# kit-cel/vae-equalizer

Measured on NVIDIA B200. Metric: DP VAE-LE train symbols/s, higher is better.
Workload: dtype f32

## Files before the change

### include/vaeq.h

```cpp
#ifndef VAEQ_H_
#define VAEQ_H_

#include <stddef.h>
#include <stdint.h>

#ifdef __cplusplus
extern "C" {
#endif

#define VAEQ_ABI_VERSION 1

#define VAEQ_OK 0
#define VAEQ_EINVAL (-1)
#define VAEQ_EWORKSPACE (-2)
#define VAEQ_ENODEV (-3)

#define VAEQ_MAX_TAPS 63
#define VAEQ_MAX_LEVELS 8

int vaeq_abi_version(void);
const char *vaeq_last_error(void);
int vaeq_sm_count(void);

#define VAEQ_K_DP_FWD 0
// ... 7 lines not shown
#define VAEQ_K_DP_BWD2 8
#define VAEQ_K_DP_BWD3 9
#define VAEQ_K_DP_FRAME 10
#define VAEQ_NKINDS 11
int vaeq_kernel_timing(int32_t enable);
int vaeq_kernel_timing_read(float *ms_sum, int32_t *count);
int64_t vaeq_launch_count(int32_t kind);

typedef struct vaeq_dp_desc {
    int32_t B;
    int32_t sps;
    int32_t M;
    int32_t n_lev;
    float nu_sc;
    int32_t flags;
    const float *rx;
    int64_t ld_rx;
    const float *amp;
    const float *P;
    const float *var;
    float *W;
    float *h;
    float *adam;
    float *q;
    int64_t ld_q;
    float *out;
    int64_t ld_out;
    float *q_keep;
    int64_t ld_q_keep;
    float *out_keep;
    int64_t ld_out_keep;
    int32_t keep_lo, keep_n;
    float *loss;
    float *var_est;
    float *gW;
    float *gh;
    void *workspace;
    size_t workspace_bytes;
} vaeq_dp_desc;

#define VAEQ_F_AMSGRAD 1

size_t vaeq_dp_workspace_bytes(int32_t B, int32_t M, int32_t n_lev);
size_t vaeq_adam_state_floats(int32_t M);

int vaeq_dp_force_generic(int32_t on);

int vaeq_dp_dynamic_tiles(int32_t on);

int vaeq_dp_tc_taps(int32_t on);

int vaeq_dp_tc_forward(int32_t on);

int vaeq_dp_forward(const vaeq_dp_desc *d, void *stream);
int vaeq_dp_forward_backward(const vaeq_dp_desc *d, void *stream);
int vaeq_dp_loss_from_q(const vaeq_dp_desc *d, float *gq, int64_t ld_gq, void *stream);

size_t vaeq_eq_backward_scratch_bytes(int32_t B, int32_t M);
int vaeq_eq_backward(const float *rx, int64_t ld_rx, const float *q, int64_t ld_q, const float *out, int64_t ld_out, const float *gq,
                     int64_t ld_gq, const float *gout, int64_t ld_gout, const float *amp, const float *var, int32_t n_lev, int32_t B,
                     int32_t M, float *gW, void *scratch, void *stream);

int vaeq_dp_train_step(const vaeq_dp_desc *d, float lr_w, float lr_h, void *stream);

int vaeq_dp_train_frame(const vaeq_dp_desc *d, int32_t n_steps, int32_t stride_sym, int32_t keep_lo_in_dst,
                        float lr_w, float lr_h, float *loss_steps, float *var_est_steps, void *stream);

int vaeq_dp_persistent_frames(int32_t mode);

size_t vaeq_dp_runs_workspace_bytes(int32_t B, int32_t M, int32_t n_lev, int32_t n_runs);
typedef struct vaeq_dp_runs {
    int32_t n_runs;
    int64_t rs_rx, rs_amp, rs_P, rs_var, rs_W, rs_h, rs_adam, rs_q, rs_out, rs_q_keep, rs_out_keep;
    const float *nu_sc;
    const float *lr_w, *lr_h;
} vaeq_dp_runs;
int vaeq_dp_train_frame_runs(const vaeq_dp_desc *d, const vaeq_dp_runs *runs, int32_t n_steps, int32_t stride_sym,
                             int32_t keep_lo_in_dst, float lr_w, float lr_h, float *loss_steps, float *var_est_steps,
                             void *stream);
int vaeq_dp_frame_runs_per_sm(int32_t per_sm);

size_t vaeq_dp_split_stats_doubles(int32_t M);
int vaeq_dp_split_forward(const vaeq_dp_desc *d, int32_t sym_lo, int32_t sym_hi, double *stats_out, void *stream);
int vaeq_dp_split_backward(const vaeq_dp_desc *d, int32_t sym_lo, int32_t sym_hi, const double *stats_in, float *grads_out,
                           void *stream);
int vaeq_dp_split_update(const vaeq_dp_desc *d, const float *grads_in, float lr_w, float lr_h, void *stream);
#define VAEQ_MAX_PEERS 8
typedef struct vaeq_peer_comm {
    int32_t rank, world;
    void *slot[VAEQ_MAX_PEERS];
    int32_t *epoch;
} vaeq_peer_comm;
size_t vaeq_peer_slot_bytes(int32_t M);
int vaeq_dp_split_step_peer(const vaeq_dp_desc *d, int32_t sym_lo, int32_t sym_hi, const vaeq_peer_comm *comm, float lr_w, float lr_h,
                            void *stream);

int vaeq_adam_update(float *param, const float *grad, float *state, int32_t n, float lr, int32_t amsgrad,
                     int32_t *step_count, int32_t bump_step, void *stream);

int vaeq_soft_dec(const float *out, int64_t ld_out, const float *var, const float *amp, float nu_sc,
                  int32_t n_lev, int32_t N, float *q, int64_t ld_q, void *stream);

int vaeq_soft_dec_runs(const float *out, const float *var, const float *amp, const float *nu_sc, int32_t n_lev, int32_t N,
                       int32_t n_runs, float *q, void *stream);

size_t vaeq_find_shift_scratch_bytes(int32_t n_shift);
// ... 106 lines not shown
```

### vae_equalizer_b200/_lib.py

```python
from __future__ import annotations

import ctypes as C
import functools
import os

_HERE = os.path.dirname(os.path.abspath(__file__))
LIB_PATH = os.path.join(_HERE, "libvaeq.so")

c_f32p = C.POINTER(C.c_float)


class VaeqError(RuntimeError):
    pass


class DpDesc(C.Structure):
    _fields_ = [
        ("B", C.c_int32), ("sps", C.c_int32), ("M", C.c_int32), ("n_lev", C.c_int32),
        ("nu_sc", C.c_float), ("flags", C.c_int32),
        ("rx", C.c_void_p), ("ld_rx", C.c_int64),
        ("amp", C.c_void_p), ("P", C.c_void_p), ("var", C.c_void_p),
        ("W", C.c_void_p), ("h", C.c_void_p), ("adam", C.c_void_p),
        ("q", C.c_void_p), ("ld_q", C.c_int64),
        ("out", C.c_void_p), ("ld_out", C.c_int64),
# ... 5 lines not shown
        ("workspace", C.c_void_p), ("workspace_bytes", C.c_size_t),
    ]


class DpRuns(C.Structure):
    _fields_ = [
        ("n_runs", C.c_int32),
        ("rs_rx", C.c_int64), ("rs_amp", C.c_int64), ("rs_P", C.c_int64), ("rs_var", C.c_int64),
        ("rs_W", C.c_int64), ("rs_h", C.c_int64), ("rs_adam", C.c_int64), ("rs_q", C.c_int64), ("rs_out", C.c_int64),
        ("rs_q_keep", C.c_int64), ("rs_out_keep", C.c_int64),
        ("nu_sc", C.c_void_p), ("lr_w", C.c_void_p), ("lr_h", C.c_void_p),
    ]


class PeerComm(C.Structure):
    _fields_ = [("rank", C.c_int32), ("world", C.c_int32), ("slot", C.c_void_p * 8), ("epoch", C.c_void_p)]


class AwgnRuns(C.Structure):
    _fields_ = [
        ("n_runs", C.c_int32),
        ("rs_rx", C.c_int64), ("rs_W", C.c_int64), ("rs_h", C.c_int64), ("rs_adam", C.c_int64), ("rs_P", C.c_int64),
        ("rs_q", C.c_int64), ("rs_out", C.c_int64), ("rs_loss", C.c_int64),
        ("lr", C.c_void_p), ("var", C.c_void_p), ("amp_mean", C.c_void_p),
    ]


class AwgnDesc(C.Structure):
    _fields_ = [
        ("B", C.c_int32), ("sps", C.c_int32), ("M", C.c_int32), ("n_lev", C.c_int32),
        ("amp_mean", C.c_float), ("var", C.c_float),
        ("rx", C.c_void_p), ("amp", C.c_void_p), ("P", C.c_void_p),
        ("W", C.c_void_p), ("h", C.c_void_p), ("adam", C.c_void_p),
        ("q", C.c_void_p), ("out", C.c_void_p), ("loss", C.c_void_p),
        ("gW", C.c_void_p), ("gh", C.c_void_p),
        ("workspace", C.c_void_p), ("workspace_bytes", C.c_size_t),
    ]


_i32, _i64, _f, _vp, _sz, _u64 = C.c_int32, C.c_int64, C.c_float, C.c_void_p, C.c_size_t, C.c_uint64
PROTOTYPES = {
    "vaeq_abi_version": (C.c_int, []),
    "vaeq_last_error": (C.c_char_p, []),
    "vaeq_sm_count": (C.c_int, []),
    "vaeq_kernel_timing": (C.c_int, [_i32]),
    "vaeq_kernel_timing_read": (C.c_int, [_vp, _vp]),
    "vaeq_launch_count": (C.c_int64, [_i32]),
    "vaeq_dp_workspace_bytes": (_sz, [_i32, _i32, _i32]),
    "vaeq_adam_state_floats": (_sz, [_i32]),
    "vaeq_dp_force_generic": (C.c_int, [_i32]),
    "vaeq_dp_dynamic_tiles": (C.c_int, [_i32]),
    "vaeq_dp_tc_taps": (C.c_int, [_i32]),
    "vaeq_dp_tc_forward": (C.c_int, [_i32]),
    "vaeq_dp_forward": (C.c_int, [C.POINTER(DpDesc), _vp]),
    "vaeq_dp_forward_backward": (C.c_int, [C.POINTER(DpDesc), _vp]),
    "vaeq_dp_loss_from_q": (C.c_int, [C.POINTER(DpDesc), _vp, _i64, _vp]),
    "vaeq_eq_backward_scratch_bytes": (_sz, [_i32, _i32]),
    "vaeq_eq_backward": (C.c_int, [_vp, _i64, _vp, _i64, _vp, _i64, _vp, _i64, _vp, _i64, _vp, _vp, _i32, _i32, _i32, _vp, _vp, _vp]),
    "vaeq_dp_train_step": (C.c_int, [C.POINTER(DpDesc), _f, _f, _vp]),
    "vaeq_dp_train_frame": (C.c_int, [C.POINTER(DpDesc), _i32, _i32, _i32, _f, _f, _vp, _vp, _vp]),
    "vaeq_dp_persistent_frames": (C.c_int, [_i32]),
    "vaeq_dp_frame_runs_per_sm": (C.c_int, [_i32]),
    "vaeq_dp_runs_workspace_bytes": (_sz, [_i32, _i32, _i32, _i32]),
    "vaeq_dp_train_frame_runs": (C.c_int, [C.POINTER(DpDesc), C.POINTER(DpRuns), _i32, _i32, _i32, _f, _f, _vp, _vp, _vp]),
    "vaeq_dp_split_stats_doubles": (_sz, [_i32]),
    "vaeq_dp_split_forward": (C.c_int, [C.POINTER(DpDesc), _i32, _i32, _vp, _vp]),
    "vaeq_dp_split_backward": (C.c_int, [C.POINTER(DpDesc), _i32, _i32, _vp, _vp, _vp]),
    "vaeq_dp_split_update": (C.c_int, [C.POINTER(DpDesc), _vp, _f, _f, _vp]),
    "vaeq_peer_slot_bytes": (_sz, [_i32]),
    "vaeq_dp_split_step_peer": (C.c_int, [C.POINTER(DpDesc), _i32, _i32, C.POINTER(PeerComm), _f, _f, _vp]),
    "vaeq_adam_update": (C.c_int, [_vp, _vp, _vp, _i32, _f, _i32, _vp, _i32, _vp]),
    "vaeq_soft_dec": (C.c_int, [_vp, _i64, _vp, _vp, _f, _i32, _i32, _vp, _i64, _vp]),
    "vaeq_find_shift_scratch_bytes": (_sz, [_i32]),
    "vaeq_find_shift": (C.c_int, [_vp, _i64, _vp, _i64, _vp, _i64, _vp, _i32, _i32, _i32, _vp, _vp, _vp, _vp, _vp]),
    "vaeq_ser_iqflip": (C.c_int, [_vp, _i64, _vp, _i64, _i32, _i32, _vp, _vp, _vp]),
    "vaeq_ser_constell": (C.c_int, [_vp, _i64, _vp, _i64, _vp, _vp, _f, _i32, _i32, _vp, _vp, _vp, _vp]),
    "vaeq_frame_eval_scratch_bytes": (_sz, [_i32, _i32]),
    "vaeq_frame_eval_runs": (C.c_int, [_vp, _i64, _i64, _vp, _i64, _i64, _vp, _i64, _i64, _vp, _vp, _i64, _vp, _i32, _i32, _i32, _i32, _i32,
                                      _i32, _i32, _vp, _vp, _vp, _vp, _vp]),
    "vaeq_frame_eval_runs_ex": (C.c_int, [_vp, _i64, _i64, _vp, _i64, _i64, _vp, _i64, _i64, _vp, _vp, _i64, _vp, _i32, _i32, _i32, _i32, _i32,
                                         _i32, _i32, _i32, _vp, _vp, _vp, _vp, _vp, _vp]),
    "vaeq_cma_align_rescale": (C.c_int, [_vp, _i64, _i64, _vp, _vp, _i32, _i32, _i32, _vp, _vp]),
    "vaeq_soft_dec_runs": (C.c_int, [_vp, _vp, _vp, _vp, _i32, _i32, _i32, _vp, _vp]),
    "vaeq_gmi": (C.c_int, [_vp, _i64, _vp, _i64, _vp, _i32, _i32, _vp, _vp, _vp]),
    "vaeq_cma_scratch_bytes": (_sz, [_i32, _i32, _i32]),
    "vaeq_cma": (C.c_int, [_i32, _vp, _i32, _f, _vp, _i32, _f, _i32, _i32, _i32, _i32, _vp, _vp, _i32, _vp, _vp]),
    "vaeq_cpe_scratch_bytes": (_sz, [_i32]),
    "vaeq_gen_levels": (C.c_int, [_vp, _vp, _i32, _i32, _i32, _i32, _u64, _vp, _vp, _i32, _vp]),
    "vaeq_gen_pulse": (C.c_int, [_vp, _vp, _i32, _i32, _vp, _i32, _vp]),
    "vaeq_gen_jones": (C.c_int, [_vp, _vp, _vp, _vp, _f, _f, _i32, _i32, _vp]),
    "vaeq_gen_noise": (C.c_int, [_vp, _vp, _u64, _i32, _i32, _vp, _i32, _vp]),
    "vaeq_cpe": (C.c_int, [_vp, _i32, _vp, _vp, _vp]),
    "vaeq_cpe_runs_scratch_bytes": (_sz, [_i32, _i32]),
    "vaeq_cpe_runs": (C.c_int, [_vp, _i32, _i32, _vp, _vp, _vp]),
    "vaeq_cma_awgn": (C.c_int, [_vp, _i32, _f, _vp, _i32, _f, _i32, _i32, _vp, _vp, _i32, _vp]),
    "vaeq_cpe_awgn": (C.c_int, [_vp, _i32, _i32, _vp, _vp, _vp]),
    "vaeq_ser_cma": (C.c_int, [_vp, _i64, _vp, _i64, _vp, _i32, _i32, _vp, _vp, _vp, _vp]),
    "vaeq_find_shift_symb": (C.c_int, [_vp, _i32, _vp, _i64, _i32, _i32, _vp, _vp, _vp]),
    "vaeq_cma_awgn_runs": (C.c_int, [_vp, _i64, _i64, _i64, _i32, _i32, _vp, _i64, _i64, _i32, _vp, _i32, _vp, _f, _i32, _vp, _i32, _vp]),
    "vaeq_awgn_cma_eval_scratch_bytes": (_sz, [_i32, _i32, _i32, _i32]),
    "vaeq_awgn_cma_eval_runs": (C.c_int, [_vp, _i64, _i64, _vp, _i64, _i64, _vp, _i32, _i32, _i32, _i32, _i32, _vp, _vp, _vp, _vp, _vp]),
    "vaeq_awgn_workspace_bytes": (_sz, [_i32, _i32, _i32]),
    "vaeq_adam_state_floats_awgn": (_sz, [_i32]),
    "vaeq_awgn_forward": (C.c_int, [C.POINTER(AwgnDesc), _vp]),
    "vaeq_awgn_forward_backward": (C.c_int, [C.POINTER(AwgnDesc), _vp]),
    "vaeq_awgn_train_step": (C.c_int, [C.POINTER(AwgnDesc), _f, _f, _vp]),
# ... 71 lines not shown
```

### vae_equalizer_b200/csrc/dp_fast.cu

```cuda
#include "dp_fast.cuh"

namespace vaeq {

template <bool SWZ = false>
__device__ __forceinline__ void load_x_phases(const DpK &p, int t0, float4 *xe, float4 *xo) {
    const int sym0 = t0 - FT_HP - FT_XOFF;
#pragma unroll 1
    for (int j = threadIdx.x; j < FT_XN / 2; j += FT_NT) {
        const int64_t s0 = 2 * (int64_t)sym0 + 4 * j;
        float4 v[4];
        if (s0 >= 0 && s0 + 3 < p.L) {
#pragma unroll
            for (int r = 0; r < 4; ++r) v[r] = __ldg(reinterpret_cast<const float4 *>(p.rx + (int64_t)r * p.ld_rx + s0));
        } else {
#pragma unroll
            for (int r = 0; r < 4; ++r) {
                float t[4];
#pragma unroll
                for (int k = 0; k < 4; ++k) {
                    const int64_t s = s0 + k;
                    t[k] = (s >= 0 && s < p.L) ? p.rx[(int64_t)r * p.ld_rx + s] : 0.f;
                }
                v[r] = make_float4(t[0], t[1], t[2], t[3]);
            }
// ... 474 lines not shown
    }

#pragma unroll
    for (int a = 0; a < RL::AMAX; ++a)
#pragma unroll
        for (int k = 0; k < 8; ++k) {
            const float2 v2 = acc2[a][2 * (k >> 2) + (k & 1)];
            const float s = warp_sum(((k >> 1) & 1) ? v2.y : v2.x);
            if (lane == 0) red[wid * (RL::AMAX * 8) + a * 8 + k] = s;
        }
    __syncthreads();
    if (wid < 4) {
        float *dst = p.gpart + (int64_t)blockIdx.x * 16 * M;
        for (int idx = lane; idx < n_real * 8; idx += 32) {
            const int a = idx >> 3, k = idx & 7, oi = k >> 1, cidx = k & 1, o = oi >> 1, i = oi & 1;
            float s = 0.f;
            if (a == BASE) {
#pragma unroll
                for (int w = 0; w < FT_NW; ++w) s += red[w * (RL::AMAX * 8) + idx];
            } else {
#pragma unroll
                for (int w = wid; w < FT_NW; w += 4) s += red[w * (RL::AMAX * 8) + idx];
            }
            const int lag = a0 + a;
            if (FAM == 1) dst[8 * M + ((o * 2 + i) * 2 + cidx) * M + (2 * MH - ph - 2 * lag)] = 2.f * p.scal[DP_KAPPA_OFF + o] * s;
            else dst[(o * 4 + 2 * cidx + i) * M + (2 * lag + ph)] = s;
        }
    }
}

template <int MH>
static size_t fast_smem_fwd() {
    return (size_t)(2 * FT_XS + FT_ES + 2 * FT_TAPV * (2 * MH + 1) + FT_RAW) * sizeof(float4) + sizeof(FastConst) + 5 * 32 * sizeof(float) + 64;
}
template <int MH>
static size_t fast_smem_bwd1() {
    return (size_t)(2 * FT_ES + FT_TAPV * (2 * MH + 1) + 12 * FT_NT) * sizeof(float4) + sizeof(FastConst) + (2 * (2 * MH + 2) + 2) * sizeof(float) + 64;
}
template <int MH, int FAM>
static size_t fast_smem_taps() {
    return (size_t)(FAM == 0 ? 2 * FT_XS + FT_RAW + 2 * 4 * FT_GROW : FT_ES + 4 * FT_GROW + 2 * 8 * FT_GROW) * sizeof(float4) +
           FT_NW * Roles<MH>::AMAX * 8 * sizeof(float) + 64;
}

template <typename K>
static int fast_prepare(K kern, size_t smem, int *grid) {
    VAEQ_CUDA(cudaFuncSetAttribute(kern, cudaFuncAttributeMaxDynamicSharedMemorySize, (int)smem));
    int per = 0;
    VAEQ_CUDA(cudaOccupancyMaxActiveBlocksPerMultiprocessor(&per, kern, FT_NT, smem));
    *grid = max(1, per) * sm_count();
    return VAEQ_OK;
}

extern bool g_tc_taps, g_tc_fwd;
template <int NL, int MH>
static int dp_run_fast_t(DpK p, int mode, cudaStream_t st, int *grid_bwd_out) {
    static int grids[VAEQ_MAX_DEVICES][4] = {{0}};
    int &gF = grids[cur_device()][0], &g1 = grids[cur_device()][1], &g2 = grids[cur_device()][2], &g3 = grids[cur_device()][3];
    const size_t sf = fast_smem_fwd<MH>(), s1 = fast_smem_bwd1<MH>(), s2 = fast_smem_taps<MH, 0>(), s3 = fast_smem_taps<MH, 1>();
    if (!gF) {
        int rc;
        if ((rc = fast_prepare(k_dp_fwd_fast<NL, MH>, sf, &gF))) return rc;
        if ((rc = fast_prepare(k_dp_bwd1_fast<NL, MH>, s1, &g1))) return rc;
        if ((rc = fast_prepare(k_dp_taps_fast<MH, 0>, s2, &g2))) return rc;
        if ((rc = fast_prepare(k_dp_taps_fast<MH, 1>, s3, &g3))) return rc;
        g2 = g3 = min(g2, g3);
    }
    p.T = FT_T;
    p.keep_vec = p.qk != nullptr && p.keep_lo % 4 == 0 && p.keep_base % 4 == 0 && p.ld_qk % 4 == 0 && p.ld_outk % 4 == 0 &&
                 (reinterpret_cast<uintptr_t>(p.qk) | reinterpret_cast<uintptr_t>(p.outk)) % 16 == 0;
    const int nt_f = (p.chi - p.clo + FT_T - 1) / FT_T, nt_b = (p.sym_hi - p.sym_lo + FT_T - 1) / FT_T;
    const int gf = min(min(gF, DP_GRID_CAP), nt_f), gb1 = min(min(g1, DP_GRID_CAP), nt_b), gt = min(min(g2, DP_GRID_CAP), nt_b);
    if (mode != DP_MODE_SPLIT_BWD) {
        p.ntiles = nt_f;
        int nparts_f = gf, rc_f = VAEQ_OK;
        if (g_tc_fwd && dp_fwd_tc_launch(p, NL, st, &nparts_f, &rc_f)) {
            if (rc_f) return rc_f;
        } else {
            ktime_begin(VAEQ_K_DP_FWD, st);
            k_dp_fwd_fast<NL, MH><<<gf, FT_NT, sf, st>>>(p);
            ktime_end(VAEQ_K_DP_FWD, st);
            VAEQ_LAUNCH_CHECK("k_dp_fwd_fast");
        }
        *grid_bwd_out = nparts_f;
        if (mode == DP_MODE_SPLIT_FWD) return VAEQ_OK;
        const int rc = dp_launch_fin(p, nparts_f, st);
        if (rc) return rc;
    }
    if (mode == DP_MODE_FWD) return VAEQ_OK;
    p.ntiles = nt_b;
    ktime_begin(VAEQ_K_DP_BWD, st);
    k_dp_bwd1_fast<NL, MH><<<gb1, FT_NT, s1, st>>>(p);
    ktime_end(VAEQ_K_DP_BWD, st);
    VAEQ_LAUNCH_CHECK("k_dp_bwd1_fast");
    if (g_tc_taps) {
        int rc = VAEQ_OK;
        if (dp_taps_tc_launch(p, st, grid_bwd_out, &rc)) return rc;
    }
    ktime_begin(VAEQ_K_DP_BWD2, st);
    k_dp_taps_fast<MH, 0><<<gt, FT_NT, s2, st>>>(p);
    ktime_end(VAEQ_K_DP_BWD2, st);
    VAEQ_LAUNCH_CHECK("k_dp_taps_fast<W>");
    ktime_begin(VAEQ_K_DP_BWD3, st);
    k_dp_taps_fast<MH, 1><<<gt, FT_NT, s3, st>>>(p);
    ktime_end(VAEQ_K_DP_BWD3, st);
    VAEQ_LAUNCH_CHECK("k_dp_taps_fast<h>");
    *grid_bwd_out = gt;
    return VAEQ_OK;
}

bool g_tc_fwd = true;

bool g_tc_taps = true;

int dp_try_fast(const DpK &p, int n_lev, int mode, cudaStream_t st, int *grid_bwd_out, int *rc) {
    const bool no_q = p.q == nullptr;
    const bool aligned = (p.B % 4 == 0) && (p.ld_rx % 4 == 0) && (no_q || ((p.ld_q % 4 == 0) && (p.ld_out % 4 == 0))) &&
                         ((reinterpret_cast<uintptr_t>(p.rx) | reinterpret_cast<uintptr_t>(p.q) | reinterpret_cast<uintptr_t>(p.out)) % 16 == 0);
    if (!aligned || p.B < 2 * FT_T) return 0;
    if ((p.sym_lo | p.sym_hi | p.clo | p.chi) % 4 != 0) return 0;
    *rc = VAEQ_OK;
#define FAST_CASE(NL_, MH_)                                             \
    if (n_lev == NL_ && p.mh == MH_) {                                  \
        *rc = dp_run_fast_t<NL_, MH_>(p, mode, st, grid_bwd_out);       \
        return 1;                                                       \
    }
    FAST_CASE(8, 12)
    FAST_CASE(8, 6)
    FAST_CASE(8, 4)
    FAST_CASE(8, 2)
    FAST_CASE(4, 12)
    FAST_CASE(2, 12)
#undef FAST_CASE
    return 0;
}

}

extern "C" int vaeq_dp_tc_forward(int32_t on) {
    vaeq::g_tc_fwd = on != 0;
    return VAEQ_OK;
}

extern "C" int vaeq_dp_tc_taps(int32_t on) {
    if (on != 0 && on != 1) {
        vaeq::set_error("vaeq_dp_tc_taps: %d is not 0 (CUDA-core kernels) or 1 (tensor cores)", on);
        return VAEQ_EINVAL;
    }
    vaeq::g_tc_taps = on != 0;
    return VAEQ_OK;
}
```

### vae_equalizer_b200/csrc/dp_fwd_tc.cu

```cuda
#include <type_traits>
#include "dp_fast.cuh"
#include "tma.cuh"

namespace vaeq {

constexpr int FC_NG = 4;
constexpr int FC_GT = 128;
constexpr int FC_NT = FC_NG * FC_GT;
constexpr int FC_XCH = 264;
constexpr int FC_XCB = 4352;
constexpr int FC_XB = 4 * FC_XCB;
constexpr int FC_QB = 8704;
static_assert(2 * FC_QB <= FC_XB && FC_QB % 512 == 0 && FC_QB >= 528 * 16, "E_q hi | lo live in the x_lo array");
static_assert(FT_TE == 4 * FC_GT, "a tile is 128 blocks of 4 symbols");

__device__ __forceinline__ uint64_t umma_desc(uint32_t saddr, uint32_t lbo, uint32_t sbo, uint32_t layout) {
    return (uint64_t)((saddr >> 4) & 0x3fff) | ((uint64_t)((lbo >> 4) & 0x3fff) << 16) | ((uint64_t)((sbo >> 4) & 0x3fff) << 32) | (1ull << 46) |
           ((uint64_t)layout << 61);
}
constexpr uint32_t UMMA_SW_NONE = 0, UMMA_SW64 = 4, UMMA_SW32 = 6;
__host__ __device__ constexpr uint32_t umma_idesc_k(int N) { return (1u << 4) | (2u << 7) | (2u << 10) | ((uint32_t)(N >> 3) << 17) | ((128u >> 4) << 24); }
__device__ __forceinline__ void umma_tf32_k(uint32_t tmem_d, uint64_t da, uint64_t db, uint32_t idesc, uint32_t acc) {
    asm volatile(
        "{\n\t.reg .pred p;\n\tsetp.ne.b32 p, %4, 0;\n\t"
        "tcgen05.mma.cta_group::1.kind::tf32 [%0], %1, %2, %3, p;\n\t}\n" ::"r"(tmem_d),
        "l"(da), "l"(db), "r"(idesc), "r"(acc)
        : "memory");
}
__device__ __forceinline__ void umma_commit_to(uint64_t *bar) {
    asm volatile("tcgen05.commit.cta_group::1.mbarrier::arrive::one.shared::cluster.b64 [%0];" ::"r"(smem_u32(bar)) : "memory");
}
__device__ __forceinline__ float tf32_lo_part(float x) {
    const float r = x - __uint_as_float(__float_as_uint(x) & 0xffffe000u);
    uint32_t o;
    asm("cvt.rna.tf32.f32 %0, %1;" : "=r"(o) : "f"(r));
    return __uint_as_float(o);
}
__device__ __forceinline__ void tmem_ld16_issue(uint32_t taddr, float (&v)[16]) {
    asm volatile("tcgen05.ld.sync.aligned.32x32b.x16.b32 {%0,%1,%2,%3,%4,%5,%6,%7,%8,%9,%10,%11,%12,%13,%14,%15}, [%16];"
                 : "=f"(v[0]), "=f"(v[1]), "=f"(v[2]), "=f"(v[3]), "=f"(v[4]), "=f"(v[5]), "=f"(v[6]), "=f"(v[7]), "=f"(v[8]), "=f"(v[9]), "=f"(v[10]),
                   "=f"(v[11]), "=f"(v[12]), "=f"(v[13]), "=f"(v[14]), "=f"(v[15])
                 : "r"(taddr));
}
__device__ __forceinline__ void tmem_ld16_wait(float (&v)[16]) {
    asm volatile("tcgen05.wait::ld.sync.aligned;"
                 : "+f"(v[0]), "+f"(v[1]), "+f"(v[2]), "+f"(v[3]), "+f"(v[4]), "+f"(v[5]), "+f"(v[6]), "+f"(v[7]), "+f"(v[8]), "+f"(v[9]), "+f"(v[10]),
                   "+f"(v[11]), "+f"(v[12]), "+f"(v[13]), "+f"(v[14]), "+f"(v[15])
                 :
                 : "memory");
}
__device__ __forceinline__ void tmem_ld16(uint32_t taddr, float (&v)[16]) {
    tmem_ld16_issue(taddr, v);
    tmem_ld16_wait(v);
}
__device__ __forceinline__ void tmem_st16(uint32_t taddr, const float (&v)[16]) {
    asm volatile("tcgen05.st.sync.aligned.32x32b.x16.b32 [%0], {%1,%2,%3,%4,%5,%6,%7,%8,%9,%10,%11,%12,%13,%14,%15,%16};" ::"r"(taddr),
                 "r"(__float_as_uint(v[0])), "r"(__float_as_uint(v[1])), "r"(__float_as_uint(v[2])), "r"(__float_as_uint(v[3])), "r"(__float_as_uint(v[4])),
                 "r"(__float_as_uint(v[5])), "r"(__float_as_uint(v[6])), "r"(__float_as_uint(v[7])), "r"(__float_as_uint(v[8])), "r"(__float_as_uint(v[9])),
                 "r"(__float_as_uint(v[10])), "r"(__float_as_uint(v[11])), "r"(__float_as_uint(v[12])), "r"(__float_as_uint(v[13])),
                 "r"(__float_as_uint(v[14])), "r"(__float_as_uint(v[15]))
                 : "memory");
}
__device__ __forceinline__ void cp_async16_zfill(void *dst_smem, const void *src_gmem, bool ok) {
    const unsigned d = (unsigned)__cvta_generic_to_shared(dst_smem);
    const int n = ok ? 16 : 0;
    asm volatile("cp.async.cg.shared.global [%0], [%1], 16, %2;" ::"r"(d), "l"(src_gmem), "r"(n) : "memory");
}
__device__ __forceinline__ uint32_t swz32(uint32_t off) { return off ^ (((off >> 7) & 1u) << 4); }
__device__ __forceinline__ uint32_t swz64(uint32_t off) { return off ^ (((off >> 7) & 3u) << 4); }

template <int MH>
struct FwdTcGeom {
    static constexpr int M = 2 * MH + 1, HF = MH / 2;
    static constexpr int OX = (MH + 3) / 4 * 4;
    static constexpr int SH = OX - MH;
    static constexpr int NKF = (6 + 2 * MH + SH) / 8 + 1;
    static constexpr int NKD = (MH + 3) / 2 + 1;
    static constexpr int TAPF_FLOATS = 4 * NKF * 256;
    static constexpr int TAPD_FLOATS = NKD * 512;
    static constexpr int FSL = (OX - 1) / 8, CSL = HF / 2;
    static_assert(FSL + 1 < NKF && CSL + 2 < NKD, "centre steps");
    __host__ __device__ static constexpr int fir_step(int t) {
        if (t < 4 * NKF) return t;
        t -= 4 * NKF;
        if (t < 4 * (NKF - 2)) {
            const int c = t / (NKF - 2 > 0 ? NKF - 2 : 1), n = t - c * (NKF - 2);
            return c * NKF + (n < FSL ? n : n + 2);
        }
        t -= 4 * (NKF - 2);
        return (t >> 1) * NKF + FSL + (t & 1);
    }
    __host__ __device__ static constexpr int conv_step(int t) {
        if (t < NKD) return t;
        t -= NKD;
        if (t < NKD - 3) return t < CSL ? t : t + 3;
        return CSL + (t - (NKD - 3));
    }
    __host__ __device__ static constexpr bool orders_are_permutations() {
        for (int st = 0; st < 4 * NKF; ++st) {
            int lo = 0, hi = 0;
            for (int t = 0; t < 8 * NKF; ++t) {
                if (fir_step(t) == st) (t < 4 * NKF ? lo : hi) += 1;
            }
            if (lo != 1 || hi != 1) return false;
        }
        for (int st = 0; st < NKD; ++st) {
            int lo = 0, hi = 0;
            for (int t = 0; t < 2 * NKD; ++t) {
                if (conv_step(t) == st) (t < NKD ? lo : hi) += 1;
            }
            if (lo != 1 || hi != 1) return false;
        }
        return true;
    }
    static constexpr size_t GROUP0 = 2048 + (size_t)(TAPF_FLOATS + TAPD_FLOATS) * 4;
    static constexpr size_t SMEM = GROUP0 + (size_t)FC_NG * 2 * FC_XB;
    static_assert(8 * 127 + 8 * NKF <= 4 * FC_XCH && 8 * 127 + OX + 8 <= 4 * FC_XCH, "sample window");
    static_assert(4 * 127 + 2 * NKD <= 528 && HF <= FT_HP - 2, "E_q window");
    static_assert(GROUP0 % 1024 == 0, "swizzled arrays need their pattern alignment");
};

template <int NL, int MH>
// ... 415 lines not shown
```

### vae_equalizer_b200/csrc/dp_kernels.cuh

```cuda
#pragma once
#include "common.cuh"

namespace vaeq {

constexpr int DP_NT = 256;
constexpr int DP_TILE = 512;
constexpr int DP_GRID_CAP = 1184;

constexpr int DP_C_OFF = 0;
constexpr int DP_KAPPA_OFF = 2;
constexpr int DP_LOSS_OFF = 4;
constexpr int DP_VAREST_OFF = 5;
constexpr int DP_S_OFF = 8;

constexpr int DP_MODE_FWD = 0, DP_MODE_FWDBWD = 1, DP_MODE_TRAIN = 2;

struct DpK {
    const float *rx;
    int64_t ld_rx;
    int B, L, M, mh, H;
    const float *amp, *P, *var;
    float nu_sc;
    float *W, *h, *adam;
    float *q;
    int64_t ld_q;
    float *out;
    int64_t ld_out;
    float *qk;
    int64_t ld_qk;
    float *outk;
    int64_t ld_outk;
    int keep_lo, keep_n;
    int64_t keep_base;
    int keep_vec;
    double *part_fwd;
    float *edge_vs;
    float *scal;
    float4 *ebuf4;
    float4 *m1buf4;
    float *erows;
    float *m1rows;
    float *gyrows;
    float *srows;
    int need_bwd;
    int from_q;
    float *gq;
    int64_t ld_gq;
    float *gpart;
    float *gfinal;
    float *loss_out, *var_est_out;
    int64_t var_est_stride;
    float *gW_out, *gh_out;
    int T, ntiles;
    int sym_lo, sym_hi, clo, chi;
    int *tile_ctr;
    int dyn;
};
constexpr int DP_SPLIT_EXT = 16;

int dp_launch_fin(const DpK &p, int nparts, cudaStream_t st);
int dp_try_fast(const DpK &p, int n_lev, int mode, cudaStream_t st, int *grid_bwd_out, int *rc);
int dp_taps_tc_launch(const DpK &p, cudaStream_t st, int *nparts, int *rc);
int dp_fwd_tc_launch(const DpK &p, int n_lev, cudaStream_t st, int *nparts, int *rc);
constexpr int DP_MODE_SPLIT_FWD = 3, DP_MODE_SPLIT_BWD = 4;

struct DpRunsK {
    int64_t rs_rx, rs_amp, rs_P, rs_var, rs_W, rs_h, rs_adam, rs_q, rs_out, rs_qk, rs_outk;
    int64_t ws_stride;
    const float *nu_sc, *lr_w, *lr_h;
    float *loss_steps, *var_steps;
    float *loss_last, *var_last, *gW_last, *gh_last;
};


constexpr int DP_SMALL_MAX_B = 1000;
size_t dp_small_smem(int B, int M);
int dp_small_launch(const DpK &p, const DpRunsK &rs, int n_lev, int n_runs, int n_steps, int stride_sym, int keep_lo_in_dst,
                    float lr_w, float lr_h, int amsgrad, cudaStream_t st);

}
```

Before: 9.532 billion.

## Move first backward DP kernel onto tcgen05 TF32 tensor cores

Adds a new backward stage-1 kernel that computes the tap-weighted error correlation as a split-precision (hi/lo) TF32 UMMA in tensor memory. Four groups per CTA overlap cp.async staging of the next tile with the current MMA, and the centre tap is handled separately on CUDA cores. The aim is to take the FIR-like accumulation off the FP32 pipes. It costs extra precision-splitting work and shared-memory swizzle staging, and it is enabled by default only for MH values 2, 4, 6 and 12. Shared UMMA helpers move into a common header.

Result: faster. 9.678 billion, median of 6 (+1.5%).

```diff
diff --git a/include/vaeq.h b/include/vaeq.h
--- a/include/vaeq.h
+++ b/include/vaeq.h
@@ -83,6 +83,8 @@
 
 int vaeq_dp_tc_forward(int32_t on);
 
+int vaeq_dp_tc_backward(int32_t on);
+
 int vaeq_dp_forward(const vaeq_dp_desc *d, void *stream);
 int vaeq_dp_forward_backward(const vaeq_dp_desc *d, void *stream);
 int vaeq_dp_loss_from_q(const vaeq_dp_desc *d, float *gq, int64_t ld_gq, void *stream);
diff --git a/vae_equalizer_b200/_lib.py b/vae_equalizer_b200/_lib.py
--- a/vae_equalizer_b200/_lib.py
+++ b/vae_equalizer_b200/_lib.py
@@ -81,6 +81,7 @@
     "vaeq_dp_dynamic_tiles": (C.c_int, [_i32]),
     "vaeq_dp_tc_taps": (C.c_int, [_i32]),
     "vaeq_dp_tc_forward": (C.c_int, [_i32]),
+    "vaeq_dp_tc_backward": (C.c_int, [_i32]),
     "vaeq_dp_forward": (C.c_int, [C.POINTER(DpDesc), _vp]),
     "vaeq_dp_forward_backward": (C.c_int, [C.POINTER(DpDesc), _vp]),
     "vaeq_dp_loss_from_q": (C.c_int, [C.POINTER(DpDesc), _vp, _i64, _vp]),
diff --git a/vae_equalizer_b200/csrc/dp_bwd1_tc.cu b/vae_equalizer_b200/csrc/dp_bwd1_tc.cu
--- /dev/null
+++ b/vae_equalizer_b200/csrc/dp_bwd1_tc.cu
@@ -0,0 +1,261 @@
+#include "dp_fast.cuh"
+#include "umma.cuh"
+
+namespace vaeq {
+
+constexpr int BC_NG = 4;
+constexpr int BC_GT = 128;
+constexpr int BC_NT = BC_NG * BC_GT;
+constexpr int BC_QB = 8704;
+constexpr int BC_SB = 8 * BC_GT * 16;
+constexpr int BC_GB = 4 * BC_QB + BC_SB;
+static_assert(FT_TE == 4 * BC_GT, "a tile is 128 blocks of 4 symbols");
+static_assert(BC_QB % 512 == 0 && BC_GB % 1024 == 0, "swizzled arrays need their pattern alignment");
+
+template <int MH>
+struct Bwd1TcGeom {
+    static constexpr int M = 2 * MH + 1, HF = MH / 2;
+    static constexpr int NKD = (MH + 3) / 2 + 1;
+    static constexpr int CSL = (HF - 1) / 2, NC = (HF + 4) / 2 - CSL + 1, NO = NKD - NC;
+    static constexpr int TAP_FLOATS = 2 * NKD * 256;
+    __host__ __device__ static constexpr int step(int t) {
+        if (t < 2 * NKD) return t;
+        t -= 2 * NKD;
+        if (t < 2 * NO) {
+            const int ph = t / (NO > 0 ? NO : 1), n = t - ph * NO;
+            return (2 + ph) * NKD + (n < CSL ? n : n + NC);
+        }
+        t -= 2 * NO;
+        const int ph = t / NC;
+        return (2 + ph) * NKD + CSL + (t - ph * NC);
+    }
+    __host__ __device__ static constexpr bool order_is_permutation() {
+        for (int s = 0; s < 4 * NKD; ++s) {
+            int n = 0;
+            for (int t = 0; t < 4 * NKD; ++t) n += step(t) == s;
+            if (n != 1) return false;
+        }
+        return true;
+    }
+    static constexpr size_t GROUP0 = 1024 + (size_t)TAP_FLOATS * 4;
+    static constexpr size_t SMEM = GROUP0 + (size_t)BC_NG * BC_GB;
+    static_assert(CSL >= 0 && NO >= 0 && 2 * CSL <= HF - 1 && 2 * (CSL + NC) >= HF + 5, "centre steps");
+    static_assert(4 * 127 + 2 * NKD <= 528 && HF <= FT_HP - 2, "e window");
+    static_assert(4 * 125 + 2 * NKD <= FT_TE + HF, "the rows of owned blocks read written positions only");
+    static_assert(GROUP0 % 1024 == 0 && SMEM <= 232448, "shared memory");
+};
+
+template <int MH>
+__global__ void __launch_bounds__(BC_NT, 1) k_dp_bwd1_tc(DpK p) {
+    using G = Bwd1TcGeom<MH>;
+    static_assert(G::order_is_permutation(), "MMA issue order");
+    constexpr int M = G::M, HF = G::HF, NKD = G::NKD;
+    extern __shared__ __align__(1024) unsigned char smem[];
+    uint64_t *bars = reinterpret_cast<uint64_t *>(smem);
+    uint32_t *tmem_slot = reinterpret_cast<uint32_t *>(smem + 32);
+    int *s_next = reinterpret_cast<int *>(smem + 64);
+    float4 *ctr = reinterpret_cast<float4 *>(smem + 128);
+    float *PSg = reinterpret_cast<float *>(smem + 256);
+    float *tap = reinterpret_cast<float *>(smem + 1024);
+    const int tid = threadIdx.x, gt = tid & 127;
+    const int warp_u = __shfl_sync(0xffffffffu, tid >> 5, 0);
+    const int g = warp_u >> 2, wq = warp_u & 3;
+    unsigned char *ea = smem + G::GROUP0 + (size_t)g * BC_GB;
+    float4 *stg = reinterpret_cast<float4 *>(ea + 4 * BC_QB);
+    const float kap0 = p.scal[DP_KAPPA_OFF], kap1 = p.scal[DP_KAPPA_OFF + 1];
+
+    for (int idx = tid; idx < G::TAP_FLOATS; idx += BC_NT) {
+        const int st = idx >> 8, rem = idx & 255, n = (rem >> 6) * 8 + ((rem & 31) >> 2), k8 = ((rem >> 5) & 1) * 4 + (rem & 3);
+        const int ph = st / NKD, pos = 2 * (st - ph * NKD) + (k8 >> 2), c = k8 & 3;
+        const int half = n >> 4, i = (n >> 2) & 3, o = n & 3, a = pos - i, j = 2 * a + ph;
+        float v = 0.f;
+        if (a >= 0 && a < (ph ? MH : MH + 1) && j != MH) {
+            const int chi = c >> 1, ic = c & 1, nu = o >> 1, oc = o & 1;
+            const float sc = 2.f * (chi ? kap1 : kap0);
+            const float tr = sc * p.h[((chi * 2 + nu) * 2 + 0) * M + j], ti = -sc * p.h[((chi * 2 + nu) * 2 + 1) * M + j];
+            v = oc == ic ? tr : (oc ? ti : -ti);
+        }
+        tap[idx] = half ? tf32_lo_part(v) : v;
+    }
+    if (tid >= 32 && tid < 48) {
+        const int c = (tid - 32) >> 2, o = tid & 3, chi = c >> 1, ic = c & 1, nu = o >> 1, oc = o & 1;
+        const float sc = 2.f * (chi ? kap1 : kap0);
+        const float tr = sc * p.h[((chi * 2 + nu) * 2 + 0) * M + MH], ti = -sc * p.h[((chi * 2 + nu) * 2 + 1) * M + MH];
+        reinterpret_cast<float *>(ctr)[c * 4 + o] = oc == ic ? tr : (oc ? ti : -ti);
+    }
+    if (tid >= 64 && tid < 66) {
+        const int nu = tid - 64;
+        float a = 0.f;
+        PSg[nu * (M + 1)] = 0.f;
+        for (int j = 0; j < M; ++j) {
+            const float h0r = p.h[((0 * 2 + nu) * 2 + 0) * M + j], h0i = p.h[((0 * 2 + nu) * 2 + 1) * M + j];
+            const float h1r = p.h[((1 * 2 + nu) * 2 + 0) * M + j], h1i = p.h[((1 * 2 + nu) * 2 + 1) * M + j];
+            a += kap0 * (h0r * h0r + h0i * h0i) + kap1 * (h1r * h1r + h1i * h1i);
+            PSg[nu * (M + 1) + j + 1] = a;
+        }
+    }
+    if (tid == 0) {
+        for (int b = 0; b < BC_NG; ++b) mbar_init(bars + b, 1);
+        asm volatile("fence.mbarrier_init.release.cluster;" ::: "memory");
+    }
+    if (tid < 32) {
+        asm volatile("tcgen05.alloc.cta_group::1.sync.aligned.shared::cta.b32 [%0], 128;" ::"r"(smem_u32(tmem_slot)) : "memory");
+        asm volatile("tcgen05.relinquish_alloc_permit.cta_group::1.sync.aligned;" ::: "memory");
+    }
+    asm volatile("fence.proxy.async.shared::cta;" ::: "memory");
+    asm volatile("tcgen05.fence::before_thread_sync;" ::: "memory");
+    __syncthreads();
+    asm volatile("tcgen05.fence::after_thread_sync;" ::: "memory");
+    const uint32_t tmem = *tmem_slot;
+
+    uint64_t *bar = bars + g;
+    const uint32_t tm_g = tmem + 32 * g + ((uint32_t)(32 * wq) << 16);
+    const int nv = (int)gridDim.x * BC_NG, vcta = (int)blockIdx.x * BC_NG + g;
+    const int i0 = FT_R * gt;
+    uint32_t par = 0;
+    auto stage_e = [&](int tile_s) {
+        const int u0 = p.sym_lo + tile_s * FT_T - FT_HP + i0;
+        const bool in_seq = (u0 >= 0) && (u0 < p.B);
+        const float *src = p.erows + (in_seq ? u0 : 0);
+#pragma unroll
+        for (int k = 0; k < 8; ++k) cp_async16_zfill(stg + k * BC_GT + gt, src + (int64_t)k * p.B, in_seq);
+        if (in_seq && (i0 >= FT_HP) && (i0 < FT_HP + FT_T) && (u0 < p.sym_hi)) {
+#pragma unroll
+            for (int k = 0; k < 12; ++k) asm volatile("prefetch.global.L2 [%0];" ::"l"(p.srows + (int64_t)k * p.B + u0));
+        }
+        asm volatile("cp.async.commit_group;" ::: "memory");
+    };
+    if (vcta < p.ntiles) stage_e(vcta);
+
+#pragma unroll 1
+    for (int tile = vcta; tile < p.ntiles; par ^= 1) {
+        const int t0 = p.sym_lo + tile * FT_T;
+        if (gt == 0) s_next[2 * g + par] = p.dyn ? atomicAdd(p.tile_ctr + 1, 1) + nv : tile + nv;
+        const int u0 = t0 - FT_HP + i0;
+        const bool in_seq = (u0 >= 0) && (u0 < p.B);
+        const bool owned = in_seq && (i0 >= FT_HP) && (i0 < FT_HP + FT_T) && (u0 < p.sym_hi);
+        asm volatile("cp.async.wait_group 0;" ::: "memory");
+        {
+            float4 er[8];
+#pragma unroll
+            for (int k = 0; k < 8; ++k) er[k] = stg[k * BC_GT + gt];
+#pragma unroll
+            for (int ph = 0; ph < 2; ++ph)
+#pragma unroll
+                for (int r = 0; r < FT_R; ++r) {
+                    const uint32_t off = swz64(16u * (i0 + r + HF));
+                    const float4 v = make_float4(f4c(er[4 * ph], r), f4c(er[4 * ph + 1], r), f4c(er[4 * ph + 2], r), f4c(er[4 * ph + 3], r));
+                    *reinterpret_cast<float4 *>(ea + (2 + ph) * BC_QB + off) = v;
+                    *reinterpret_cast<float4 *>(ea + ph * BC_QB + off) = make_float4(tf32_lo_part(v.x), tf32_lo_part(v.y), tf32_lo_part(v.z), tf32_lo_part(v.w));
+                }
+        }
+        asm volatile("fence.proxy.async.shared::cta;" ::: "memory");
+        asm volatile("tcgen05.fence::before_thread_sync;" ::: "memory");
+        named_bar_sync(1 + g, BC_GT);
+        const int tile_next = s_next[2 * g + par];
+        if (gt == 0) {
+            asm volatile("tcgen05.fence::after_thread_sync;" ::: "memory");
+            const uint64_t da0 = umma_desc(smem_u32(ea), 16, 512, UMMA_SW64), db0 = umma_desc(smem_u32(tap), 128, 256, UMMA_SW_NONE);
+#pragma unroll
+            for (int t = 0; t < 4 * NKD; ++t) {
+                const int st = G::step(t), ar = st / NKD, s = st - ar * NKD;
+                const uint64_t ao = (uint64_t)((ar * BC_QB + 32 * s) >> 4), bo = (uint64_t)((((ar & 1) * NKD + s) * 1024) >> 4);
+                umma_tf32_k(tmem + 32 * g, da0 + ao, db0 + bo, umma_idesc_k(32), t != 0);
+            }
+            umma_commit_to(bar);
+        }
+        __syncwarp();
+        if (tile_next < p.ntiles) stage_e(tile_next);
+        float4 sc[12];
+        if (owned) {
+#pragma unroll
+            for (int k = 0; k < 12; ++k) sc[k] = ld_row4(p.srows, p.B, k, u0);
+        }
+        float2 gc[FT_R][2];
+#pragma unroll
+        for (int r = 0; r < FT_R; ++r) {
+            const float4 e = *reinterpret_cast<const float4 *>(ea + 2 * BC_QB + swz64(16u * (i0 + r + HF)));
+            float2 a0 = make_float2(0.f, 0.f), a1 = a0;
+#pragma unroll
+            for (int ci = 0; ci < 4; ++ci) {
+                const float4 w = ctr[ci];
+                const float ev = f4c(e, ci);
+                a0 = __ffma2_rn(make_float2(w.x, w.y), make_float2(ev, ev), a0);
+                a1 = __ffma2_rn(make_float2(w.z, w.w), make_float2(ev, ev), a1);
+            }
+            gc[r][0] = a0;
+            gc[r][1] = a1;
+        }
+        mbar_wait(bar, par);
+        asm volatile("tcgen05.fence::after_thread_sync;" ::: "memory");
+        float vh[16], vl[16];
+        tmem_ld16_issue(tm_g, vh);
+        tmem_ld16_issue(tm_g + 16, vl);
+        tmem_ld16_wait(vh);
+        tmem_ld16_wait(vl);
+        if (owned) {
+            float entw[FT_R];
+#pragma unroll
+            for (int r = 0; r < FT_R; ++r) {
+                const int u = u0 + r;
+                entw[r] = (u >= MH && u < p.B - MH) ? LN2 : 0.f;
+            }
+#pragma unroll
+            for (int pol = 0; pol < 2; ++pol) {
+                float gV[FT_R];
+#pragma unroll
+                for (int r = 0; r < FT_R; ++r) {
+                    const int u = u0 + r;
+                    const int jlo = max(0, 2 * MH - 2 * u), jhi = min(M, p.L - 2 * u);
+                    gV[r] = PSg[pol * (M + 1) + jhi] - PSg[pol * (M + 1) + jlo];
+                }
+#pragma unroll
+                for (int cq = 0; cq < 2; ++cq) {
+                    const int cc = 2 * pol + cq;
+                    const float4 s1 = sc[cc], t2 = sc[4 + cc], s3 = sc[8 + cc];
+                    float gy[FT_R];
+#pragma unroll
+                    for (int r = 0; r < FT_R; ++r) {
+                        const float gE = (vh[4 * r + cc] + vl[4 * r + cc]) + (cq ? gc[r][pol].y : gc[r][pol].x);
+                        gy[r] = fmaf(gE, f4c(s1, r), fmaf(gV[r], f4c(t2, r), entw[r] * f4c(s3, r)));
+                    }
+                    st_row4(p.gyrows, p.B, cc, u0, make_float4(gy[0], gy[1], gy[2], gy[3]));
+                }
+            }
+        }
+        tile = tile_next;
+    }
+
+    asm volatile("tcgen05.fence::before_thread_sync;" ::: "memory");
+    __syncthreads();
+    if (tid < 32) asm volatile("tcgen05.dealloc.cta_group::1.sync.aligned.b32 %0, 128;" ::"r"(*tmem_slot) : "memory");
+}
+
+template <int MH>
+static int bwd1_tc_launch_t(DpK p, cudaStream_t st) {
+    static SmemAttrCache set;
+    using G = Bwd1TcGeom<MH>;
+    if (int rc = ensure_dyn_smem(k_dp_bwd1_tc<MH>, G::SMEM, set)) return rc;
+    const int nvc = min(BC_NG * sm_count(), p.ntiles), grid = (nvc + BC_NG - 1) / BC_NG;
+    ktime_begin(VAEQ_K_DP_BWD, st);
+    k_dp_bwd1_tc<MH><<<grid, BC_NT, G::SMEM, st>>>(p);
+    ktime_end(VAEQ_K_DP_BWD, st);
+    VAEQ_LAUNCH_CHECK("k_dp_bwd1_tc");
+    return VAEQ_OK;
+}
+
+int dp_bwd1_tc_launch(const DpK &p, cudaStream_t st, int *rc) {
+#define TC_CASE(MH_)                                \
+    if (p.mh == MH_) {                              \
+        *rc = bwd1_tc_launch_t<MH_>(p, st);         \
+        return 1;                                   \
+    }
+    TC_CASE(12)
+    TC_CASE(6)
+    TC_CASE(4)
+    TC_CASE(2)
+#undef TC_CASE
+    return 0;
+}
+
+}
diff --git a/vae_equalizer_b200/csrc/dp_fast.cu b/vae_equalizer_b200/csrc/dp_fast.cu
--- a/vae_equalizer_b200/csrc/dp_fast.cu
+++ b/vae_equalizer_b200/csrc/dp_fast.cu
@@ -550,7 +550,7 @@
     return VAEQ_OK;
 }
 
-extern bool g_tc_taps, g_tc_fwd;
+extern bool g_tc_taps, g_tc_fwd, g_tc_bwd;
 template <int NL, int MH>
 static int dp_run_fast_t(DpK p, int mode, cudaStream_t st, int *grid_bwd_out) {
     static int grids[VAEQ_MAX_DEVICES][4] = {{0}};
@@ -587,10 +587,15 @@
     }
     if (mode == DP_MODE_FWD) return VAEQ_OK;
     p.ntiles = nt_b;
-    ktime_begin(VAEQ_K_DP_BWD, st);
-    k_dp_bwd1_fast<NL, MH><<<gb1, FT_NT, s1, st>>>(p);
-    ktime_end(VAEQ_K_DP_BWD, st);
-    VAEQ_LAUNCH_CHECK("k_dp_bwd1_fast");
+    int rc_b = VAEQ_OK;
+    if (g_tc_bwd && dp_bwd1_tc_launch(p, st, &rc_b)) {
+        if (rc_b) return rc_b;
+    } else {
+        ktime_begin(VAEQ_K_DP_BWD, st);
+        k_dp_bwd1_fast<NL, MH><<<gb1, FT_NT, s1, st>>>(p);
+        ktime_end(VAEQ_K_DP_BWD, st);
+        VAEQ_LAUNCH_CHECK("k_dp_bwd1_fast");
+    }
     if (g_tc_taps) {
         int rc = VAEQ_OK;
         if (dp_taps_tc_launch(p, st, grid_bwd_out, &rc)) return rc;
@@ -610,6 +615,8 @@
 bool g_tc_fwd = true;
 
 bool g_tc_taps = true;
+
+bool g_tc_bwd = true;
 
 int dp_try_fast(const DpK &p, int n_lev, int mode, cudaStream_t st, int *grid_bwd_out, int *rc) {
     const bool no_q = p.q == nullptr;
@@ -648,3 +655,12 @@
     vaeq::g_tc_taps = on != 0;
     return VAEQ_OK;
 }
+
+extern "C" int vaeq_dp_tc_backward(int32_t on) {
+    if (on != 0 && on != 1) {
+        vaeq::set_error("vaeq_dp_tc_backward: %d is not 0 (CUDA-core kernel) or 1 (tensor cores)", on);
+        return VAEQ_EINVAL;
+    }
+    vaeq::g_tc_bwd = on != 0;
+    return VAEQ_OK;
+}
diff --git a/vae_equalizer_b200/csrc/dp_fwd_tc.cu b/vae_equalizer_b200/csrc/dp_fwd_tc.cu
--- a/vae_equalizer_b200/csrc/dp_fwd_tc.cu
+++ b/vae_equalizer_b200/csrc/dp_fwd_tc.cu
@@ -1,6 +1,6 @@
 #include <type_traits>
 #include "dp_fast.cuh"
-#include "tma.cuh"
+#include "umma.cuh"
 
 namespace vaeq {
 
@@ -14,45 +14,6 @@
 static_assert(2 * FC_QB <= FC_XB && FC_QB % 512 == 0 && FC_QB >= 528 * 16, "E_q hi | lo live in the x_lo array");
 static_assert(FT_TE == 4 * FC_GT, "a tile is 128 blocks of 4 symbols");
 
-__device__ __forceinline__ uint64_t umma_desc(uint32_t saddr, uint32_t lbo, uint32_t sbo, uint32_t layout) {
-    return (uint64_t)((saddr >> 4) & 0x3fff) | ((uint64_t)((lbo >> 4) & 0x3fff) << 16) | ((uint64_t)((sbo >> 4) & 0x3fff) << 32) | (1ull << 46) |
-           ((uint64_t)layout << 61);
-}
-constexpr uint32_t UMMA_SW_NONE = 0, UMMA_SW64 = 4, UMMA_SW32 = 6;
-__host__ __device__ constexpr uint32_t umma_idesc_k(int N) { return (1u << 4) | (2u << 7) | (2u << 10) | ((uint32_t)(N >> 3) << 17) | ((128u >> 4) << 24); }
-__device__ __forceinline__ void umma_tf32_k(uint32_t tmem_d, uint64_t da, uint64_t db, uint32_t idesc, uint32_t acc) {
-    asm volatile(
-        "{\n\t.reg .pred p;\n\tsetp.ne.b32 p, %4, 0;\n\t"
-        "tcgen05.mma.cta_group::1.kind::tf32 [%0], %1, %2, %3, p;\n\t}\n" ::"r"(tmem_d),
-        "l"(da), "l"(db), "r"(idesc), "r"(acc)
-        : "memory");
-}
-__device__ __forceinline__ void umma_commit_to(uint64_t *bar) {
-    asm volatile("tcgen05.commit.cta_group::1.mbarrier::arrive::one.shared::cluster.b64 [%0];" ::"r"(smem_u32(bar)) : "memory");
-}
-__device__ __forceinline__ float tf32_lo_part(float x) {
-    const float r = x - __uint_as_float(__float_as_uint(x) & 0xffffe000u);
-    uint32_t o;
-    asm("cvt.rna.tf32.f32 %0, %1;" : "=r"(o) : "f"(r));
-    return __uint_as_float(o);
-}
-__device__ __forceinline__ void tmem_ld16_issue(uint32_t taddr, float (&v)[16]) {
-    asm volatile("tcgen05.ld.sync.aligned.32x32b.x16.b32 {%0,%1,%2,%3,%4,%5,%6,%7,%8,%9,%10,%11,%12,%13,%14,%15}, [%16];"
-                 : "=f"(v[0]), "=f"(v[1]), "=f"(v[2]), "=f"(v[3]), "=f"(v[4]), "=f"(v[5]), "=f"(v[6]), "=f"(v[7]), "=f"(v[8]), "=f"(v[9]), "=f"(v[10]),
-                   "=f"(v[11]), "=f"(v[12]), "=f"(v[13]), "=f"(v[14]), "=f"(v[15])
-                 : "r"(taddr));
-}
-__device__ __forceinline__ void tmem_ld16_wait(float (&v)[16]) {
-    asm volatile("tcgen05.wait::ld.sync.aligned;"
-                 : "+f"(v[0]), "+f"(v[1]), "+f"(v[2]), "+f"(v[3]), "+f"(v[4]), "+f"(v[5]), "+f"(v[6]), "+f"(v[7]), "+f"(v[8]), "+f"(v[9]), "+f"(v[10]),
-                   "+f"(v[11]), "+f"(v[12]), "+f"(v[13]), "+f"(v[14]), "+f"(v[15])
-                 :
-                 : "memory");
-}
-__device__ __forceinline__ void tmem_ld16(uint32_t taddr, float (&v)[16]) {
-    tmem_ld16_issue(taddr, v);
-    tmem_ld16_wait(v);
-}
 __device__ __forceinline__ void tmem_st16(uint32_t taddr, const float (&v)[16]) {
     asm volatile("tcgen05.st.sync.aligned.32x32b.x16.b32 [%0], {%1,%2,%3,%4,%5,%6,%7,%8,%9,%10,%11,%12,%13,%14,%15,%16};" ::"r"(taddr),
                  "r"(__float_as_uint(v[0])), "r"(__float_as_uint(v[1])), "r"(__float_as_uint(v[2])), "r"(__float_as_uint(v[3])), "r"(__float_as_uint(v[4])),
@@ -61,13 +22,7 @@
                  "r"(__float_as_uint(v[14])), "r"(__float_as_uint(v[15]))
                  : "memory");
 }
-__device__ __forceinline__ void cp_async16_zfill(void *dst_smem, const void *src_gmem, bool ok) {
-    const unsigned d = (unsigned)__cvta_generic_to_shared(dst_smem);
-    const int n = ok ? 16 : 0;
-    asm volatile("cp.async.cg.shared.global [%0], [%1], 16, %2;" ::"r"(d), "l"(src_gmem), "r"(n) : "memory");
-}
 __device__ __forceinline__ uint32_t swz32(uint32_t off) { return off ^ (((off >> 7) & 1u) << 4); }
-__device__ __forceinline__ uint32_t swz64(uint32_t off) { return off ^ (((off >> 7) & 3u) << 4); }
 
 template <int MH>
 struct FwdTcGeom {
diff --git a/vae_equalizer_b200/csrc/dp_kernels.cuh b/vae_equalizer_b200/csrc/dp_kernels.cuh
--- a/vae_equalizer_b200/csrc/dp_kernels.cuh
+++ b/vae_equalizer_b200/csrc/dp_kernels.cuh
@@ -62,6 +62,7 @@
 int dp_try_fast(const DpK &p, int n_lev, int mode, cudaStream_t st, int *grid_bwd_out, int *rc);
 int dp_taps_tc_launch(const DpK &p, cudaStream_t st, int *nparts, int *rc);
 int dp_fwd_tc_launch(const DpK &p, int n_lev, cudaStream_t st, int *nparts, int *rc);
+int dp_bwd1_tc_launch(const DpK &p, cudaStream_t st, int *rc);
 constexpr int DP_MODE_SPLIT_FWD = 3, DP_MODE_SPLIT_BWD = 4;
 
 struct DpRunsK {
diff --git a/vae_equalizer_b200/csrc/umma.cuh b/vae_equalizer_b200/csrc/umma.cuh
--- /dev/null
+++ b/vae_equalizer_b200/csrc/umma.cuh
@@ -0,0 +1,52 @@
+#pragma once
+#include "tma.cuh"
+
+namespace vaeq {
+
+__device__ __forceinline__ uint64_t umma_desc(uint32_t saddr, uint32_t lbo, uint32_t sbo, uint32_t layout) {
+    return (uint64_t)((saddr >> 4) & 0x3fff) | ((uint64_t)((lbo >> 4) & 0x3fff) << 16) | ((uint64_t)((sbo >> 4) & 0x3fff) << 32) | (1ull << 46) |
+           ((uint64_t)layout << 61);
+}
+constexpr uint32_t UMMA_SW_NONE = 0, UMMA_SW64 = 4, UMMA_SW32 = 6;
+__host__ __device__ constexpr uint32_t umma_idesc_k(int N) { return (1u << 4) | (2u << 7) | (2u << 10) | ((uint32_t)(N >> 3) << 17) | ((128u >> 4) << 24); }
+__device__ __forceinline__ void umma_tf32_k(uint32_t tmem_d, uint64_t da, uint64_t db, uint32_t idesc, uint32_t acc) {
+    asm volatile(
+        "{\n\t.reg .pred p;\n\tsetp.ne.b32 p, %4, 0;\n\t"
+        "tcgen05.mma.cta_group::1.kind::tf32 [%0], %1, %2, %3, p;\n\t}\n" ::"r"(tmem_d),
+        "l"(da), "l"(db), "r"(idesc), "r"(acc)
+        : "memory");
+}
+__device__ __forceinline__ void umma_commit_to(uint64_t *bar) {
+    asm volatile("tcgen05.commit.cta_group::1.mbarrier::arrive::one.shared::cluster.b64 [%0];" ::"r"(smem_u32(bar)) : "memory");
+}
+__device__ __forceinline__ float tf32_lo_part(float x) {
+    const float r = x - __uint_as_float(__float_as_uint(x) & 0xffffe000u);
+    uint32_t o;
+    asm("cvt.rna.tf32.f32 %0, %1;" : "=r"(o) : "f"(r));
+    return __uint_as_float(o);
+}
+__device__ __forceinline__ void tmem_ld16_issue(uint32_t taddr, float (&v)[16]) {
+    asm volatile("tcgen05.ld.sync.aligned.32x32b.x16.b32 {%0,%1,%2,%3,%4,%5,%6,%7,%8,%9,%10,%11,%12,%13,%14,%15}, [%16];"
+                 : "=f"(v[0]), "=f"(v[1]), "=f"(v[2]), "=f"(v[3]), "=f"(v[4]), "=f"(v[5]), "=f"(v[6]), "=f"(v[7]), "=f"(v[8]), "=f"(v[9]), "=f"(v[10]),
+                   "=f"(v[11]), "=f"(v[12]), "=f"(v[13]), "=f"(v[14]), "=f"(v[15])
+                 : "r"(taddr));
+}
+__device__ __forceinline__ void tmem_ld16_wait(float (&v)[16]) {
+    asm volatile("tcgen05.wait::ld.sync.aligned;"
+                 : "+f"(v[0]), "+f"(v[1]), "+f"(v[2]), "+f"(v[3]), "+f"(v[4]), "+f"(v[5]), "+f"(v[6]), "+f"(v[7]), "+f"(v[8]), "+f"(v[9]), "+f"(v[10]),
+                   "+f"(v[11]), "+f"(v[12]), "+f"(v[13]), "+f"(v[14]), "+f"(v[15])
+                 :
+                 : "memory");
+}
+__device__ __forceinline__ void tmem_ld16(uint32_t taddr, float (&v)[16]) {
+    tmem_ld16_issue(taddr, v);
+    tmem_ld16_wait(v);
+}
+__device__ __forceinline__ void cp_async16_zfill(void *dst_smem, const void *src_gmem, bool ok) {
+    const unsigned d = (unsigned)__cvta_generic_to_shared(dst_smem);
+    const int n = ok ? 16 : 0;
+    asm volatile("cp.async.cg.shared.global [%0], [%1], 16, %2;" ::"r"(d), "l"(src_gmem), "r"(n) : "memory");
+}
+__device__ __forceinline__ uint32_t swz64(uint32_t off) { return off ^ (((off >> 7) & 3u) << 4); }
+
+}
```
